# Brummi/BehindTheScenes

Measured on AMD Instinct MI355X. Metric: rendered rays/sec (192x640x64 samples), higher is better.
Workload: dtype f32 (lin_in as 3-term f16 split products on the f16 MFMA, f32 accumulate; everything else f32); 1 GPU; KITTI eval_depth.yaml forward, bs=1/GPU, 192x640, 2 views x 122880 rays, 64 samples/ray, nv=1, learn_empty=True (the yaml's effective default), want_weights+alphas, renderer only (feature-map encoder stand-in); samples_per_ray=64, parallelism=frames x1

## Files before the change

behindthescenes_amd/csrc/bts_common.h:

```cpp
#pragma once
#include <hip/hip_runtime.h>
#include <stdint.h>

#include "../../include/bts_render.h"

typedef float f32x16 __attribute__((ext_vector_type(16)));
typedef float f32x4 __attribute__((ext_vector_type(4)));
typedef float f32x2 __attribute__((ext_vector_type(2)));

#define BTS_EPS 1e-3f

namespace bts {

constexpr int kFwdWaves = 2;

constexpr int kNumFreqs = 6;
constexpr int kPeDim = 3 + 6 * kNumFreqs;

__device__ __forceinline__ void swap32(float& a, float& b) {
  auto r = __builtin_amdgcn_permlane32_swap(__float_as_uint(a), __float_as_uint(b), false, false);
  a = __uint_as_float(r[0]);
  b = __uint_as_float(r[1]);
}

// ... 157 lines not shown
  Taps t;
  t.w00 = (ex - ix) * (ey - iy);
  t.w01 = (ix - fx) * (ey - iy);
  t.w10 = (ex - ix) * (iy - fy);
  t.w11 = (ix - fx) * (iy - fy);
  x0 = (int)fx, y0 = (int)fy;
  x1 = min(x0 + 1, W - 1), y1 = min(y0 + 1, H - 1);
  x0 = max(0, min(x0, W - 1));
  y0 = max(0, min(y0, H - 1));
  x0 >>= fs, x1 >>= fs, y0 >>= fs, y1 >>= fs, W >>= fs;
  t.o00 = y0 * W + x0;
  t.o01 = y0 * W + x1;
  t.o10 = y1 * W + x0;
  t.o11 = y1 * W + x1;
  return t;
}

__device__ __forceinline__ Taps make_taps(float x, float y, int H, int W, int fs = 0) {
  int x0, y0, x1, y1;
  return make_taps_xy(x, y, H, W, x0, y0, x1, y1, fs);
}

__host__ __device__ inline int tile_cols(int Hm, int Wm, int blocks) { return (blocks && (Hm & 3) == 0 && (Wm & 15) == 0) ? (Wm >> 4) : 0; }
__device__ __forceinline__ unsigned tile_of(int y, int x, int Wm, int tw) {
  return tw ? (unsigned)((y >> 2) * tw + (x >> 4)) : (unsigned)(y * Wm + x) >> 6;
}
__device__ __forceinline__ int tile_base(int t, int Wm, int tw) {
  if (!tw) return t * 64;
  const int ty = t / tw;
  return ty * 4 * Wm + (t - ty * tw) * 16;
}
__device__ __forceinline__ int tile_rs(int Wm, int tw) { return tw ? Wm - 16 : 0; }
__device__ __forceinline__ int tile_px(int p0, int i, int rs) { return p0 + i + (i >> 4) * rs; }
__device__ __forceinline__ int tile_px_c(int p0, int cslot, int lslot, int rs) { return p0 + cslot + (cslot >> 4) * rs + lslot; }

__device__ __forceinline__ float depth_code(const Proj& pe, bool by_distance, bool inv_z, float inv_dmax, float inv_range, float d_min, float range) {
  const float v = by_distance ? pe.dist : pe.z;
  float r;
  if (inv_z) {
    const float vc = fmaxf(v, BTS_EPS);
    const float rv = div_by(1.0f, vc, by_distance ? __builtin_amdgcn_rcpf(vc) : pe.rz);
    r = div_by(rv - inv_dmax, inv_range, rcp_nr(inv_range));
  } else {
    r = div_by(v - d_min, range, rcp_nr(range));
  }
  return __builtin_fmaf(2.0f, r, -1.0f);
}

__device__ __forceinline__ float linspace_at(float start, float end, int steps, int i) {
  const float step = (end - start) / (float)(steps - 1);
  return i < steps / 2 ? start + step * (float)i : end - step * (float)(steps - i - 1);
}
__device__ __forceinline__ float coarse_base(int K, int k) { return K > 1 ? linspace_at(0.0f, 1.0f - 1.0f / (float)K, K, k) : 0.0f; }
__device__ __forceinline__ float coarse_depth(float u, float base, float step, float near, float far, bool lindisp) {
  const float sv = base + u * step;
  if (!lindisp) return near * (1.0f - sv) + far * sv;
  const float inv_near = div_by(1.0f, near, __builtin_amdgcn_rcpf(near)), inv_far = div_by(1.0f, far, __builtin_amdgcn_rcpf(far));
  const float den = inv_near * (1.0f - sv) + inv_far * sv;
  return div_by(1.0f, den, __builtin_amdgcn_rcpf(den));
}

template <int I>
__device__ __forceinline__ float pe_entry(const float (&v)[3], float freq_factor) {
  if constexpr (I < 3) {
    return v[I];
  } else if constexpr (I < kPeDim) {
    constexpr int j = I - 3;
    constexpr int oct = j / 6;
    constexpr int within = j % 6;
    constexpr int comp = within % 3;
    constexpr bool is_cos = within >= 3;
    const float f = freq_factor * (float)(1 << oct);
    float arg = v[comp] * f;
    if constexpr (is_cos) arg = arg + 1.57079637050628662109375f;
    return sinf(arg);
  } else if constexpr (I == kPeDim) {
    return 1.0f;
  } else {
    return 0.0f;
  }
}

__device__ __forceinline__ float relu1(float x) { return __builtin_amdgcn_fmed3f(x, 0.0f, 3.4028234663852886e38f); }

__device__ __forceinline__ int xcd_remap(int b, int nwg) {
  const int q = nwg >> 3, r = nwg & 7;
  const int xcd = b & 7, idx = b >> 3;
  return (xcd < r ? xcd * (q + 1) : r * (q + 1) + (xcd - r) * q) + idx;
}

__host__ __device__ constexpr int proj_storage_index(int hid) {
  const int ht = hid >> 5, r = hid & 31;
  const int q = r >> 3, h = (r >> 2) & 1, e = r & 3;
  return ht * 32 + h * 16 + q * 4 + e;
}
__host__ __device__ constexpr int proj_hidden_of_storage(int s) {
  const int ht = s >> 5, r = s & 31;
  const int h = r >> 4, q = (r >> 2) & 3, e = r & 3;
  return ht * 32 + 8 * q + 4 * h + e;
}

struct MlpLayout {
  int d_in, hd, nb;
  __host__ __device__ int w_in() const { return 0; }
  __host__ __device__ int b_in() const { return hd * d_in; }
  __host__ __device__ int blk(int i) const { return hd * d_in + hd + i * (2 * hd * hd + 2 * hd); }
  __host__ __device__ int blk_w0(int i) const { return blk(i); }
  __host__ __device__ int blk_b0(int i) const { return blk(i) + hd * hd; }
  __host__ __device__ int blk_w1(int i) const { return blk(i) + hd * hd + hd; }
  __host__ __device__ int blk_b1(int i) const { return blk(i) + 2 * hd * hd + hd; }
  __host__ __device__ int w_out() const { return blk(nb); }
  __host__ __device__ int b_out() const { return blk(nb) + hd; }
  __host__ __device__ int total() const { return blk(nb) + hd + 1; }
};

}
```

behindthescenes_amd/csrc/bts_field_kernel.h:

```cpp
#pragma once
#include "bts_common.h"
#include "bts_host.h"

#include <cstdio>
#include <cstring>

namespace bts {

struct FwdParams {
  const float* feat;
  const float* proj;
  const float* K_enc;
  const float* w2c_enc;
  const float* imgs;
  const float* K_r;
  const float* w2c_r;
  const float* empty_feature;
  const float* mlp;
  int n, H, W, nv;
  int fs;
  int enc_view;
  int code_mode, inv_z, learn_empty, empty_empty;
  float freq_factor, d_min, d_max;
  float inv_dmax, inv_range, range;
  const float* rays;
  const float* z_samp;
  const float* jitter;
  float* z_out;
  int lindisp;
  int Bp, K, hard_cap, white_bkgd;
  float* rgb;
  float* depth;
  float* weights;
  float* alphas;
  float* invalid;
  float* rgb_samps;
  float* sigma_raw;
  float* trans;
  float* invalid_wsum;
  float* invalid_any;
  const float* sigma_noise;
  union {
    const float* xyz;
    unsigned* sched;
  };
  union {
    float* q_sigma;
    const float* mlp_image;
  };
  int only_density;
  int tiles_per_sample;
  unsigned long long* dbg;
  int ablate;
  int lpr;
  int chunk_log2;
  int dyn_first;
  long groups;
};

struct PinnedSet {
  static constexpr int K = 64, nv = 1, fs = 0, enc_view = 0, lindisp = 1, empty_empty = 0, white_bkgd = 0;
  static constexpr int code_mode = 0, inv_z = 1, learn_empty = 1, hard_cap = 1;
  static bool matches(const FwdParams& p) {
    return p.lpr == 64 && p.K == K && p.nv == nv && p.fs == fs && p.enc_view == enc_view && !p.z_samp && p.jitter && !p.z_out && p.lindisp != 0 &&
           !p.sigma_noise && p.empty_empty == 0 && p.white_bkgd == 0 && p.code_mode == code_mode && p.inv_z != 0 && p.learn_empty != 0 &&
           p.hard_cap != 0 && p.rgb && p.depth && p.weights && p.alphas && p.invalid && !p.rgb_samps && !p.sigma_raw && !p.trans &&
           !p.invalid_wsum && !p.invalid_any;
  }
};

#ifdef BTS_PROBE
#define BTS_ABL(bit) ((p.ablate & (bit)) != 0)
#else
#define BTS_ABL(bit) false
#endif

template <int C, int HD, int NB, bool PROJ>
struct Lds {
  static constexpr int CF = PROJ ? 0 : C;
  static constexpr int KIN = CF + kPeDim + 1;
  static constexpr int W_IN = 0;
  static constexpr int BLK = W_IN + KIN * HD;
  static constexpr int BLK_STRIDE = 2 * HD * HD + 2 * HD;
  static constexpr int W_OUT = BLK + NB * BLK_STRIDE;
  static constexpr int EMPTY = W_OUT + HD;
  static constexpr int TOTAL = EMPTY + (PROJ ? HD : C);
};

template <int C>
__host__ __device__ constexpr int kernel_to_ref_input(int k) {
  if (k < C + 2) return k;
  if (k == C + 2) return C + 2;
  if (k == C + 3) return -1;
  return k - 1;
}

template <int C, int HD, int NB, bool PROJ>
__device__ __forceinline__ void stage_weights(float* lds, const float* __restrict__ mlp, const float* __restrict__ empty) {
  using L = Lds<C, HD, NB, PROJ>;
  constexpr int D_IN = C + kPeDim;
  const MlpLayout ml{D_IN, HD, NB};
  for (int i = threadIdx.x; i < L::KIN * HD; i += blockDim.x) {
    const int k = i / HD, hid = i % HD;
    const int src = kernel_to_ref_input<C>(k + (PROJ ? C : 0));
    lds[L::W_IN + i] = src >= 0 ? mlp[ml.w_in() + hid * D_IN + src] : mlp[ml.b_in() + hid];
  }
#pragma unroll
  for (int b = 0; b < NB; ++b) {
    float* base = lds + L::BLK + b * L::BLK_STRIDE;
    for (int i = threadIdx.x; i < HD * HD; i += blockDim.x) {
      const int k = i / HD, out = i % HD;
      base[i] = mlp[ml.blk_w0(b) + out * HD + k];
      base[HD * HD + HD + i] = mlp[ml.blk_w1(b) + out * HD + k];
    }
    for (int i = threadIdx.x; i < HD; i += blockDim.x) {
      base[HD * HD + i] = mlp[ml.blk_b0(b) + i];
      base[2 * HD * HD + HD + i] = mlp[ml.blk_b1(b) + i];
    }
  }
  for (int i = threadIdx.x; i < HD; i += blockDim.x) lds[L::W_OUT + i] = mlp[ml.w_out() + i];
  if constexpr (PROJ) {
    for (int hid = threadIdx.x; hid < HD; hid += blockDim.x) {
      float a = 0.0f;
      if (empty)
        for (int c = 0; c < C; ++c) a = __builtin_fmaf(mlp[ml.w_in() + hid * D_IN + c], empty[c], a);
      lds[L::EMPTY + hid] = a;
    }
  } else {
    for (int i = threadIdx.x; i < C; i += blockDim.x) lds[L::EMPTY + i] = empty ? empty[i] : 0.0f;
  }
}

struct GBuf {
  float4 v[2][4];
};

template <int HD>
__device__ __forceinline__ void gload(GBuf& b, const float4* __restrict__ G, const int (&o)[4], int tp2, int idx4) {
#pragma unroll
  for (int t = 0; t < 2; ++t) {
    const float4* row = G + (long)o[2 * tp2 + t] * (HD / 4) + idx4;
#pragma unroll
    for (int q = 0; q < 4; ++q) b.v[t][q] = row[q];
  }
}


template <bool FIRST>
__device__ __forceinline__ void gblend(f32x16& acc, const GBuf& b, float w0, float w1) {
  const f32x2 w0v = {w0, w0}, w1v = {w1, w1};
// ... 620 lines not shown
```

behindthescenes_amd/csrc/bts_render_iter.h:

```cpp
{
    constexpr bool SHARED = kTwoLoops && (BTS_ITER_SHARED);
    bool other_loop = false;
    const float nrec_in = nrec, z_pre_in = z_pre, zn_pre_in = zn_pre;
    auto q = kernarg_view<FwdParams>();
    asm volatile("" : "+s"(q));
    IterHead ih(q);
    const int K = BTS_PIN(PinnedSet::K, ih.K), H = ih.H, W = ih.W, nv = BTS_PIN(PinnedSet::nv, ih.nv), fs = BTS_PIN(PinnedSet::fs, ih.fs);
    long ray = lane_ray(g, 0);
    while (g >= sample_end) ++sample, sample_end += groups_per_sample;
    const Cam enc = load_cam(ih.w2c_enc + sample * 16, ih.K_enc + sample * 9);
    const float4* __restrict__ G = reinterpret_cast<const float4*>(ih.proj) + (long)sample * (H >> fs) * (W >> fs) * (HD / 4);
    float ox, oy, oz, dx, dy, dz, near = 0.0f, far = 0.0f;
    const bool from_jitter = BTS_PIN(true, ih.z_samp == nullptr);
    if constexpr (ONE_RAY) {
      ox = lane_value(nrec, 0), oy = lane_value(nrec, 1), oz = lane_value(nrec, 2), dx = lane_value(nrec, 3), dy = lane_value(nrec, 4);
      dz = lane_value(nrec, 5), near = lane_value(nrec, 6), far = lane_value(nrec, 7);
    } else {
      const float4 r0 = reinterpret_cast<const float4*>(ih.rays)[ray * 2];
      const float4 r1 = reinterpret_cast<const float4*>(ih.rays)[ray * 2 + 1];
      ox = r0.x, oy = r0.y, oz = r0.z, dx = r0.w, dy = r1.x, dz = r1.y, near = r1.z, far = r1.w;
    }
    const float* zsrc = from_jitter ? ih.jitter : ih.z_samp;
    const float* zrow = zsrc + ray * K;
    float z_cur = z_pre, zn_cur = zn_pre;
// ... 115 lines not shown
      } else {
        __builtin_amdgcn_fence(__ATOMIC_RELEASE, "wavefront");
        __builtin_amdgcn_wave_barrier();
        gl.tab[lane * 3 + 0] = (unsigned)tp.o00 * (HD * 4u), gl.tab[lane * 3 + 1] = (unsigned)tp.o01 * (HD * 4u), gl.tab[lane * 3 + 2] = (unsigned)tp.o10 * (HD * 4u);
        __builtin_amdgcn_fence(__ATOMIC_RELEASE, "wavefront");
        __builtin_amdgcn_wave_barrier();
        __builtin_amdgcn_fence(__ATOMIC_ACQUIRE, "wavefront");
        gl_prologue<HD, PINNED>(gl, rows, G, off_next, &taps);
      }
      {
        f32x16 bias[HT];
        {
          const float* bl = lh + LH::W_RAW + 3 * HD + 4 * h;
#pragma unroll
          for (int ht = 0; ht < HT; ++ht)
#pragma unroll
            for (int j = 0; j < 4; ++j) {
              const float4 v = *reinterpret_cast<const float4*>(bl + ht * 32 + 8 * j);
              bias[ht][4 * j + 0] = v.x, bias[ht][4 * j + 1] = v.y, bias[ht][4 * j + 2] = v.z, bias[ht][4 * j + 3] = v.w;
            }
        }
        SinCos3 raw;
        pe_direct(raw, v3, ih.freq_factor);
        __builtin_amdgcn_sched_barrier(0);
        int lane4 = lane * 4;
        asm volatile("" : "+v"(lane4));
        region_seq_l<HD, 0, SHARED, PINNED>(acc, gl, rows, G, wq, off_next, lh + LH::W_F16 + lane4, LH::TERM_STRIDE, raw, v3, ih.freq_factor, bias, h, &taps);
        if constexpr (NS > kNumFreqs) {
          g_step<HD, 12, SHARED, PINNED>(acc, gl, rows, G, wq, off_next, h, &taps), g_step<HD, 13, SHARED, PINNED>(acc, gl, rows, G, wq, off_next, h, &taps);
          g_step<HD, 14, SHARED, PINNED>(acc, gl, rows, G, wq, off_next, h, &taps), g_step<HD, 15, SHARED, PINNED>(acc, gl, rows, G, wq, off_next, h, &taps);
        }
      }
      if (BTS_PIN(PinnedSet::learn_empty, q->learn_empty) && __any(use_empty)) {
#pragma unroll
        for (int ht = 0; ht < HT; ++ht)
#pragma unroll
          for (int q = 0; q < 16; ++q) {
            const float ev = lh[LH::EMPTY + ht * 32 + mfma_row(q, 0) + 4 * h];
#pragma unroll
            for (int pt = 0; pt < 2; ++pt) acc[ht][pt][q] += emp[pt] ? ev : 0.0f;
          }
      }

      int lane4b = lane * 4;
      asm volatile("" : "+v"(lane4b));
#pragma unroll
      for (int b = 0; b < NB; ++b) {
        const float* base = lds + L::BLK + b * L::BLK_STRIDE;
        f32x16 net[HT][2];
#pragma unroll
        for (int ot = 0; ot < HT; ++ot)
#pragma unroll
          for (int q = 0; q < 16; ++q) {
            const int row = ot * 32 + mfma_row(q, 0) + 4 * h;
            const float bias = lh[LH::BIAS + b * 2 * HD + row];
            net[ot][0][q] = bias, net[ot][1][q] = bias;
          }
        if constexpr (HD == 32) hidden_layer_h(net, acc, lh + LH::W_BLK + (2 * b) * LH::BLK_LAYER_STRIDE + lane4b, LH::BLK_TERM_STRIDE, inv_scale);
        else hidden_layer<HD>(net, acc, base, lane);
#pragma unroll
        for (int ot = 0; ot < HT; ++ot)
#pragma unroll
          for (int q = 0; q < 16; ++q) {
            const int row = ot * 32 + mfma_row(q, 0) + 4 * h;
            const float bias = lh[LH::BIAS + b * 2 * HD + HD + row];
            acc[ot][0][q] += bias, acc[ot][1][q] += bias;
          }
        if constexpr (HD == 32) hidden_layer_h(acc, net, lh + LH::W_BLK + (2 * b + 1) * LH::BLK_LAYER_STRIDE + lane4b, LH::BLK_TERM_STRIDE, inv_scale);
        else hidden_layer<HD>(acc, net, base + HD * HD + HD, lane);
      }

      BTS_TICK(1)
      float p0 = 0.0f, p1 = 0.0f;
      if (BTS_ABL(32)) {
#pragma unroll
        for (int ht = 0; ht < HT; ++ht) p0 += acc[ht][0][0] + acc[ht][0][5] + acc[ht][0][15], p1 += acc[ht][1][0] + acc[ht][1][5] + acc[ht][1][15];
      } else {
        f32x2 pp = {0.0f, 0.0f};
#pragma unroll
        for (int ht = 0; ht < HT; ++ht)
#pragma unroll
          for (int q = 0; q < 16; ++q) {
            const float w2 = lds[L::W_OUT + ht * 32 + mfma_row(q, 0) + 4 * h];
            pp = __builtin_elementwise_fma((f32x2){w2, w2}, (f32x2){relu1(acc[ht][0][q]), relu1(acc[ht][1][q])}, pp);
          }
        p0 = pp[0], p1 = pp[1];
      }
      swap32(p0, p1);
      s_raw = __builtin_fmaf(p0 + p1, inv_scale, b_out);
      }
      float sigma = softplus(s_raw);
      if (BTS_PIN(PinnedSet::empty_empty, q->empty_empty)) sigma = pe.invalid ? 0.0f : sigma;
      if (BTS_PIN(false, q->sigma_noise != nullptr)) sigma += q->sigma_noise[ray * K + min(k, K - 1)];
      BTS_TICK(2)

      o_rgb = (OutP)q->rgb, o_depth = (OutP)q->depth, white_bkgd = BTS_PIN(PinnedSet::white_bkgd, q->white_bkgd);
      OutP o_weights = (OutP)q->weights, o_alphas = (OutP)q->alphas, o_invalid = (OutP)q->invalid;
      float *o_rgb_samps = BTS_PIN((float*)nullptr, q->rgb_samps), *o_sigma_raw = BTS_PIN((float*)nullptr, q->sigma_raw);
      float *o_trans = BTS_PIN((float*)nullptr, q->trans), *o_iw = BTS_PIN((float*)nullptr, q->invalid_wsum), *o_ia = BTS_PIN((float*)nullptr, q->invalid_any);
      if constexpr (PINNED) asm volatile("" : "+s"(o_rgb), "+s"(o_depth), "+s"(o_weights), "+s"(o_alphas), "+s"(o_invalid));
      else
      asm volatile("" : "+s"(o_rgb), "+s"(o_depth), "+s"(o_weights), "+s"(o_alphas), "+s"(o_invalid), "+s"(o_rgb_samps), "+s"(o_sigma_raw), "+s"(o_trans),
                   "+s"(o_iw), "+s"(o_ia));

#pragma unroll
      for (int j = 0; j < NVMAX; ++j) col[3 * j] = col[3 * j + 1] = col[3 * j + 2] = 0.0f, inv[j] = pe.invalid;
      if (nv > 0 && !BTS_ABL(8)) {
#pragma unroll
        for (int j0 = 0; j0 < NVMAX; j0 += 4) {
          constexpr int NB4 = NVMAX < 4 ? NVMAX : 4;
          Taps tcs[NB4];
          bool invs[NB4];
#pragma unroll
          for (int b = 0; b < NB4; ++b) {
            const int jj = min(j0 + b, nv - 1);
            tcs[b] = tp_enc, invs[b] = pe.invalid;
            if (jj != BTS_PIN(PinnedSet::enc_view, q->enc_view)) {
              const Cam cj = load_cam(q->w2c_r + ((long)sample * nv + jj) * 16, q->K_r + ((long)sample * nv + jj) * 9);
              const Proj pc = project<false>(cj, px, py, pz);
              tcs[b] = make_taps(pc.x, pc.y, H, W);
              invs[b] = pc.invalid | pe.invalid;
            }
          }
          float4 tex[NB4][4];
#pragma unroll
          for (int b = 0; b < NB4; ++b) {
            const float4* img = reinterpret_cast<const float4*>(q->imgs) + ((long)sample * nv + min(j0 + b, nv - 1)) * H * W;
            tex[b][0] = img[tcs[b].o00], tex[b][1] = img[tcs[b].o01], tex[b][2] = img[tcs[b].o10], tex[b][3] = img[tcs[b].o11];
          }
          if constexpr (NB4 > 1) __builtin_amdgcn_sched_barrier(0);
#pragma unroll
          for (int b = 0; b < NB4; ++b) {
            const int j = j0 + b;
            const Taps& tc = tcs[b];
            const float4 a = tex[b][0], bb = tex[b][1], cc = tex[b][2], d = tex[b][3];
            const float c0 = ((a.x * tc.w00 + bb.x * tc.w01) + cc.x * tc.w10) + d.x * tc.w11;
            const float c1 = ((a.y * tc.w00 + bb.y * tc.w01) + cc.y * tc.w10) + d.y * tc.w11;
            const float c2 = ((a.z * tc.w00 + bb.z * tc.w01) + cc.z * tc.w10) + d.z * tc.w11;
            if (j < nv) col[3 * j + 0] = c0, col[3 * j + 1] = c1, col[3 * j + 2] = c2, inv[j] = invs[b];
          }
        }
      }

      const float delta = (k + 1 < K) ? (z_nx - z) : 1e10f;
      float alpha = 1.0f - transmittance(delta, sigma);
      if (BTS_PIN(PinnedSet::hard_cap, q->hard_cap) && k == K - 1) alpha = 1.0f;
      const float t = valid ? (1.0f - alpha) + 1e-10f : 1.0f;
      const float incl = seg_scan_mul(t, lpr, kl);
      float excl = dpp_f<kDppWaveShr1>(1.0f, incl);
      if (kl == 0) excl = 1.0f;
      const float T = (pk48 ? (mainl ? 1.0f : Tc_D) : T_carry) * excl;
      if (pk48) Tc_D = Tc_D * __builtin_bit_cast(float, __builtin_amdgcn_readlane(__builtin_bit_cast(int, incl), 63));
      if (ONE_RAY && K > 64) T_carry = T_carry * __builtin_bit_cast(float, __builtin_amdgcn_readlane(__builtin_bit_cast(int, incl), 63));
      const float wgt = valid ? alpha * T : 0.0f;
      BTS_TICK(3)
      if constexpr (EPI) {
        float ws[NVMAX], any[NVMAX];
        const unsigned long long seg = pk48 ? (mainl ? 0x0000FFFFFFFFFFFFull : 0xFFFF000000000000ull)
                                            : (lpr == 64 ? ~0ull : (((1ull << lpr) - 1ull) << ((lane | (lpr - 1)) - (lpr - 1))));
#pragma unroll
        for (int j = 0; j < NVMAX; ++j) {
          ws[j] = seg_scan_add((valid && inv[j]) ? wgt : 0.0f, lpr, kl);
          const unsigned long long hit = __ballot(valid && inv[j]);
          any[j] = (hit & seg) ? 1.0f : 0.0f;
        }
        if (pk48 ? (lane == 47 || lane == 63) : kl == lpr - 1) {
          const bool more = pk48 ? (!mainl && it > 0) : kc > 0;
          const long idx = ray * nv;
          if (nv == NVMAX && NVMAX % 4 == 0 && !more) {
#pragma unroll
            for (int j4 = 0; j4 < NVMAX / 4; ++j4) {
              if (o_iw) reinterpret_cast<float4*>(o_iw + idx)[j4] = make_float4(ws[4 * j4], ws[4 * j4 + 1], ws[4 * j4 + 2], ws[4 * j4 + 3]);
              if (o_ia) reinterpret_cast<float4*>(o_ia + idx)[j4] = make_float4(any[4 * j4], any[4 * j4 + 1], any[4 * j4 + 2], any[4 * j4 + 3]);
            }
          } else {
#pragma unroll
            for (int j = 0; j < NVMAX; ++j)
              if (j < nv) {
                if (o_iw) o_iw[idx + j] = (more ? o_iw[idx + j] : 0.0f) + ws[j];
                if (o_ia) o_ia[idx + j] = more ? fmaxf(o_ia[idx + j], any[j]) : any[j];
              }
          }
        }
      }
      depth_part = depth_part + wgt * z;
      w_part = w_part + wgt;
#pragma unroll
      for (int i = 0; i < NVMAX * 3; ++i) rgb_part[i] = rgb_part[i] + wgt * col[i];
      if (valid && !BTS_ABL(16)) {
        const long pk = ray * K + k;
        if constexpr (PINNED) {
          __builtin_nontemporal_store(wgt, &(o_weights + ray * K)[(unsigned)k]), __builtin_nontemporal_store(alpha, &(o_alphas + ray * K)[(unsigned)k]);
          __builtin_nontemporal_store(inv[0] ? 1.0f : 0.0f, &(o_invalid + ray * K)[(unsigned)k]);
        }
        if (BTS_PIN(false, o_weights != nullptr)) o_weights[pk] = wgt;
        if (BTS_PIN(false, o_alphas != nullptr)) o_alphas[pk] = alpha;
        if (o_sigma_raw) o_sigma_raw[pk] = s_raw;
        if (o_trans) o_trans[pk] = T;
        if (BTS_PIN(false, o_invalid != nullptr)) {
#pragma unroll
          for (int j = 0; j < NVMAX; ++j)
            if (j < nv) o_invalid[pk * nv + j] = inv[j] ? 1.0f : 0.0f;
        }
        if (o_rgb_samps) {
          float* dst = o_rgb_samps + pk * (nv * 3);
          if (nv == NVMAX && (NVMAX * 3) % 4 == 0) {
#pragma unroll
            for (int i = 0; i < NVMAX * 3 / 4; ++i)
              reinterpret_cast<float4*>(dst)[i] = make_float4(col[4 * i], col[4 * i + 1], col[4 * i + 2], col[4 * i + 3]);
          } else if (nv == NVMAX && (NVMAX * 3) % 2 == 0) {
#pragma unroll
            for (int i = 0; i < NVMAX * 3 / 2; ++i) reinterpret_cast<float2*>(dst)[i] = make_float2(col[2 * i], col[2 * i + 1]);
          } else {
#pragma unroll
            for (int i = 0; i < NVMAX * 3; ++i)
              if (i < nv * 3) dst[i] = col[i];
          }
        }
      }
      if (pk48) {
        const float dsum = seg_scan_add(depth_part, 48, kl), wsum = seg_scan_add(w_part, 48, kl);
        float csum[NVMAX * 3];
#pragma unroll
        for (int i = 0; i < NVMAX * 3; ++i) csum[i] = i < nv * 3 ? seg_scan_add(rgb_part[i], 48, kl) : 0.0f;
        if (lane == 47 || (lane == 63 && it == 2)) {
          o_depth[ray] = dsum;
#pragma unroll
          for (int i = 0; i < NVMAX * 3; ++i)
            if (i < nv * 3) o_rgb[ray * nv * 3 + i] = white_bkgd ? (csum[i] + 1.0f) - wsum : csum[i];
        }
      }
// ... 31 lines not shown
```

behindthescenes_amd/csrc/bts_render_kernel.h:

```cpp
#pragma once
#include "bts_field_kernel.h"

namespace bts {

#ifdef BTS_PROBE
#define BTS_TICK(i)                                                  \
  if (p.ablate & 128) {                                              \
    const unsigned long long t_now = __builtin_readcyclecounter();   \
    t_acc[i] += t_now - t_last;                                      \
    t_last = t_now;                                                  \
  }
#else
#define BTS_TICK(i)
#endif

template <int CTRL, int ROW_MASK = 0xF>
__device__ __forceinline__ float dpp_f(float old, float src) {
  return __builtin_bit_cast(float, __builtin_amdgcn_update_dpp(__builtin_bit_cast(int, old), __builtin_bit_cast(int, src), CTRL,
                                                               ROW_MASK, 0xF, false));
}
constexpr int kDppRowShr = 0x110;
constexpr int kDppWaveShr1 = 0x138;
constexpr int kDppWaveShl1 = 0x130;
constexpr int kDppBcast15 = 0x142;
constexpr int kDppBcast31 = 0x143;

__device__ __forceinline__ float seg_scan_mul(float x, int lpr, int kl) {
  float y;
  if (lpr == 48) {
    x *= dpp_f<kDppRowShr + 1>(1.0f, x);
    x *= dpp_f<kDppRowShr + 2>(1.0f, x);
    x *= dpp_f<kDppRowShr + 4>(1.0f, x);
    x *= dpp_f<kDppRowShr + 8>(1.0f, x);
    x *= dpp_f<kDppBcast15, 0x2>(1.0f, x);
    x *= dpp_f<kDppBcast31, 0x4>(1.0f, x);
    return x;
  }
  if (lpr >= 16) {
    x *= dpp_f<kDppRowShr + 1>(1.0f, x);
    x *= dpp_f<kDppRowShr + 2>(1.0f, x);
    x *= dpp_f<kDppRowShr + 4>(1.0f, x);
    x *= dpp_f<kDppRowShr + 8>(1.0f, x);
  } else {
    y = dpp_f<kDppRowShr + 1>(1.0f, x), x *= (kl >= 1) ? y : 1.0f;
    y = dpp_f<kDppRowShr + 2>(1.0f, x), x *= (kl >= 2) ? y : 1.0f;
    y = dpp_f<kDppRowShr + 4>(1.0f, x), x *= (kl >= 4) ? y : 1.0f;
  }
  if (lpr >= 32) x *= dpp_f<kDppBcast15, 0xA>(1.0f, x);
  if (lpr >= 64) x *= dpp_f<kDppBcast31, 0xC>(1.0f, x);
  return x;
}
__device__ __forceinline__ float seg_scan_add(float x, int lpr, int kl) {
  float y;
  if (lpr == 48) {
    x += dpp_f<kDppRowShr + 1>(0.0f, x);
    x += dpp_f<kDppRowShr + 2>(0.0f, x);
    x += dpp_f<kDppRowShr + 4>(0.0f, x);
    x += dpp_f<kDppRowShr + 8>(0.0f, x);
    x += dpp_f<kDppBcast15, 0x2>(0.0f, x);
    x += dpp_f<kDppBcast31, 0x4>(0.0f, x);
    return x;
  }
  if (lpr >= 16) {
    x += dpp_f<kDppRowShr + 1>(0.0f, x);
    x += dpp_f<kDppRowShr + 2>(0.0f, x);
    x += dpp_f<kDppRowShr + 4>(0.0f, x);
    x += dpp_f<kDppRowShr + 8>(0.0f, x);
  } else {
    y = dpp_f<kDppRowShr + 1>(0.0f, x), x += (kl >= 1) ? y : 0.0f;
    y = dpp_f<kDppRowShr + 2>(0.0f, x), x += (kl >= 2) ? y : 0.0f;
    y = dpp_f<kDppRowShr + 4>(0.0f, x), x += (kl >= 4) ? y : 0.0f;
  }
  if (lpr >= 32) x += dpp_f<kDppBcast15, 0xA>(0.0f, x);
  if (lpr >= 64) x += dpp_f<kDppBcast31, 0xC>(0.0f, x);
  return x;
}

typedef _Float16 h8 __attribute__((ext_vector_type(8)));
typedef unsigned u32x4 __attribute__((ext_vector_type(4)));

template <int C, int HD, int NB>
struct LdsH {
  static constexpr int HT = HD / 32;
  static constexpr int W_RAW = 0;
  static constexpr int W_F16 = W_RAW + 4 * HD;
  static constexpr int TERM_STRIDE = 3 * HT * 64 * 4;
  static constexpr int BIAS = W_F16 + 2 * TERM_STRIDE;
  static constexpr int EMPTY = BIAS + NB * 2 * HD;
  static constexpr int SCALE = EMPTY + HD;
  static constexpr int W_BLK = SCALE + 4;
  static constexpr int BLK_TERM_STRIDE = 2 * 64 * 4;
  static constexpr int BLK_LAYER_STRIDE = 2 * BLK_TERM_STRIDE;
  static constexpr int TOTAL = W_BLK + NB * 2 * BLK_LAYER_STRIDE;
};

template <int C, int HD, int NB>
__device__ __forceinline__ void stage_weights_h(float* lh, const float* empty_proj, const float* __restrict__ mlp) {
  using LH = LdsH<C, HD, NB>;
  constexpr int HT = HD / 32;
  constexpr int D_IN = C + kPeDim;
  const MlpLayout ml{D_IN, HD, NB};
  int* mx = reinterpret_cast<int*>(lh + LH::SCALE + 2);
  if (threadIdx.x == 0) *mx = 0;
  __syncthreads();
  float m = 0.0f;
  for (int i = threadIdx.x; i < 39 * HD; i += blockDim.x) m = fmaxf(m, fabsf(mlp[ml.w_in() + (i % HD) * D_IN + C + i / HD]));
  for (int i = threadIdx.x; i < NB * 2 * HD * HD; i += blockDim.x) {
    const int b = i / (2 * HD * HD), j = i % (2 * HD * HD);
    m = fmaxf(m, fabsf(mlp[(j < HD * HD ? ml.blk_w0(b) : ml.blk_w1(b)) + j % (HD * HD)]));
  }
  atomicMax(mx, __float_as_int(m));
  __syncthreads();
  const float wmax = __int_as_float(*mx);
  int ex = 0;
  if (wmax > 0.0f && wmax < 3.0e38f) frexpf(wmax, &ex);
  const int S = max(-40, min(40, 14 - ex));
  const float scale = ldexpf(1.0f, S);
  if (threadIdx.x == 0) lh[LH::SCALE] = scale, lh[LH::SCALE + 1] = ldexpf(1.0f, -S);
  for (int i = threadIdx.x; i < 4 * HD; i += blockDim.x) {
    const int k = i / HD, hid = i % HD;
    lh[LH::W_RAW + i] = (k < 3 ? mlp[ml.w_in() + hid * D_IN + C + k] : mlp[ml.b_in() + hid]) * scale;
  }
  _Float16* wf = reinterpret_cast<_Float16*>(lh + LH::W_F16);
  for (int i = threadIdx.x; i < 3 * HT * 64 * 8; i += blockDim.x) {
    const int e = i & 7, lane = (i >> 3) & 63, ht = (i >> 9) % HT, r = i / (HT * 512);
    const int slot = 8 * (lane >> 5) + e, hid = ht * 32 + (lane & 31);
    float w = 0.0f;
    if (slot < 12) w = mlp[ml.w_in() + hid * D_IN + C + 3 + 6 * (2 * r + slot / 6) + slot % 6] * scale;
    else if (r == 0 && slot < 14) w = mlp[ml.w_in() + hid * D_IN + C + (slot - 12)] * scale;
    else if (r == 1 && slot == 12) w = mlp[ml.w_in() + hid * D_IN + C + 2] * scale;
    asm("" : "+v"(w));
    const _Float16 hi = (_Float16)w;
// ... 362 lines not shown
template <int HD, int R, bool SH = false, bool PIN = false>
__device__ __forceinline__ void region_seq_l(f32x16 (&acc)[HD / 32][2], const GatherLds& gl, GRows& rows, const float4* __restrict__ G,
                                             const float (&wq)[2][4], unsigned (&off_next)[4], const float* wf, int term_stride, SinCos3& raw,
                                             const float (&v3)[3], float ff, const f32x16* bias, int h = 0, GTapRegs* taps = nullptr) {
  static_assert(R == 0, "entered at region 0");
  SinCos3 pre;
  region_seq_li<HD, 0, SH, PIN>(acc, gl, rows, G, wq, off_next, wf, term_stride, raw, pre, v3, ff, bias, h, taps);
}

template <int C, int HD, int NB>
__device__ __attribute__((noinline)) float eval_point_exact(const float* lds, const float4* G, const float* w2c, const float* Kc, int H, int W,
                                                            int fs, int code_mode, int inv_z, float inv_dmax, float inv_range, float d_min, float range,
                                                            float freq_factor, int learn_empty, float b_out, float px, float py, float pz) {
  FwdParams q;
  q.H = H, q.W = W, q.fs = fs, q.code_mode = code_mode, q.inv_z = inv_z, q.inv_dmax = inv_dmax, q.inv_range = inv_range, q.d_min = d_min;
  q.range = range, q.freq_factor = freq_factor, q.learn_empty = learn_empty, q.ablate = 0;
  const Cam enc = load_cam(w2c, Kc);
  Proj pe;
  return eval_point<C, HD, NB, true>(q, lds, enc, G, (int)(threadIdx.x & 63), b_out, px, py, pz, pe);
}

template <bool PIN>
struct IterHeadT {
  const float* w2c_enc;
  const float* K_enc;
  const float* proj;
  const float* rays;
  const float* z_samp;
  const float* jitter;
  int K, H, W, nv, fs, code_mode, inv_z, learn_empty;
  float inv_dmax, inv_range, d_min, range, freq_factor;
  template <typename Q>
  __device__ __forceinline__ explicit IterHeadT(Q q) {
    const FwdParams __attribute__((address_space(4)))* f = head_of(q);
    w2c_enc = f->w2c_enc, K_enc = f->K_enc, proj = f->proj, rays = f->rays, z_samp = f->z_samp, jitter = f->jitter;
    K = f->K, H = f->H, W = f->W, nv = f->nv, fs = f->fs, code_mode = f->code_mode, inv_z = f->inv_z, learn_empty = f->learn_empty;
    inv_dmax = f->inv_dmax, inv_range = f->inv_range, d_min = f->d_min, range = f->range, freq_factor = f->freq_factor;
    if constexpr (PIN)
    asm volatile("" : "+s"(w2c_enc), "+s"(K_enc), "+s"(proj), "+s"(rays), "+s"(z_samp), "+s"(K), "+s"(H), "+s"(W), "+s"(nv), "+s"(fs),
                 "+s"(code_mode), "+s"(inv_z), "+s"(learn_empty), "+s"(inv_dmax), "+s"(inv_range), "+s"(d_min), "+s"(range), "+s"(freq_factor));
  }
  static __device__ __forceinline__ const FwdParams __attribute__((address_space(4)))* head_of(const FwdParams __attribute__((address_space(4)))* q) { return q; }
  template <typename B>
  static __device__ __forceinline__ const FwdParams __attribute__((address_space(4)))* head_of(const B __attribute__((address_space(4)))* q) { return &q->f; }
};
using IterHead = IterHeadT<false>;

__device__ __forceinline__ void store4(float* p, const float4& v) { *reinterpret_cast<float4*>(p) = v; }
__device__ __forceinline__ void store4(float __attribute__((address_space(1)))* p, const float4& v) {
  *(f32x4 __attribute__((address_space(1)))*)p = (f32x4){v.x, v.y, v.z, v.w};
}

#define BTS_PIN(constant, field) (PINNED ? (constant) : (field))
template <int C, int HD, int NB, int NVMAX, bool ONE_RAY, bool F16, bool EPI = false, bool DYN = false, bool IMG = false, bool PINNED = false>
__global__ __launch_bounds__(256, kFwdWaves) void render_kernel_p(const FwdParams p) {
  static_assert(F16, "lin_in runs on the f16 matrix pipe in split precision: the fp32-input-MFMA form of rounds 1 - 2 is gone (git history)");
  static_assert(!PINNED || (ONE_RAY && !EPI && DYN && IMG && NB == 0 && NVMAX == PinnedSet::nv), "the pinned set is the evaluation frame's");
  using OutP = std::conditional_t<PINNED, float __attribute__((address_space(1)))*, float*>;
  using L = Lds<C, HD, NB, true>;
  using LH = LdsH<C, HD, NB>;
  constexpr int HT = HD / 32;
  constexpr int NS = 4 * HT;
  __shared__ __attribute__((aligned(16))) float lds[L::TOTAL + LH::TOTAL + 4];
  float* const lh = lds + ((L::TOTAL + 3) & ~3);
#ifdef BTS_PROBE
  const unsigned long long t_entry = __builtin_readcyclecounter();
#endif
  if constexpr (IMG) {
    const float4* src = reinterpret_cast<const float4*>(p.mlp_image);
    float4* dst = reinterpret_cast<float4*>(lds);
    for (int i = threadIdx.x; i < MlpImage<C, HD, NB>::FLOATS / 4; i += 256) dst[i] = src[i];
    __syncthreads();
  } else {
    stage_weights<C, HD, NB, true>(lds, p.mlp, p.empty_feature);
    __syncthreads();
    stage_weights_h<C, HD, NB>(lh, lds + L::EMPTY, p.mlp);
    __syncthreads();
  }
#ifdef BTS_PROBE
  const unsigned long long t_stage = __builtin_readcyclecounter() - t_entry;
#endif
  const float scale = __builtin_bit_cast(float, __builtin_amdgcn_readfirstlane(__builtin_bit_cast(int, lh[LH::SCALE])));
  const float inv_scale = __builtin_bit_cast(float, __builtin_amdgcn_readfirstlane(__builtin_bit_cast(int, lh[LH::SCALE + 1])));

  const int lane = threadIdx.x & 63;
  const int h0 = lane >> 5;
  const int wave = __builtin_amdgcn_readfirstlane(threadIdx.x >> 6);
  extern __shared__ __attribute__((aligned(128))) char gather_lds[];
  GatherLds gl;
  {
    char* base = gather_lds + wave * kGatherLdsPerWave;
    gl.ring = base;
    gl.ring_m0 = (unsigned)(unsigned long)base;
    gl.tab = reinterpret_cast<unsigned*>(base + 3 * 4096);
    gl.m = lane >> 3;
    gl.piece16 = 16u * (unsigned)(((lane & 7) + (lane >> 4)) & 7);
    gl.piece16x = gl.piece16 ^ 64u;
    const int col = lane & 31;
#pragma unroll
    for (int q = 0; q < 4; ++q) gl.rd[q] = (unsigned)(col * 128 + ((4 * h0 + q - (col >> 1)) & 7) * 16);
  }
  const int nwg = gridDim.x;
  const int wg = xcd_remap(blockIdx.x, nwg);
  const int wg_per_xcd = nwg >> 3;
  const int xcd = wg / wg_per_xcd;
  const int lw = (wg - xcd * wg_per_xcd) * 4 + wave;
  const int waves_per_xcd = wg_per_xcd * 4;
  const int lpr = ONE_RAY ? 64 : p.lpr;
  const bool pk48 = !ONE_RAY && lpr == 48;
  const bool mainl = lane < 48;
  const int R = pk48 ? 4 : 64 / lpr;
  const int kl = pk48 ? (mainl ? lane : lane - 48) : lane & (lpr - 1);
  auto lane_ray = [&](int gg, int it) -> long { return pk48 ? (long)gg * 4 + (mainl ? it : 3) : (long)gg * R + lane / lpr; };
  auto lane_k = [&](int it) -> int { return pk48 && !mainl ? 16 * it + kl : kl; };
  const int CHL = p.chunk_log2;
  const int n_groups = (int)p.groups;
  const int n_chunks = (n_groups + (1 << CHL) - 1) >> CHL;
  auto group_of = [&](int idx) -> int {
    const int c = ((idx >> CHL) << 3) + xcd;
    const int gg = (c << CHL) + (idx & ((1 << CHL) - 1));
    return (c < n_chunks && gg < n_groups) ? gg : -1;
  };
  const int Bp = p.Bp;
  const float b_out = as_const(p.mlp)[MlpLayout{C + kPeDim, HD, NB}.b_out()];
  const int lane_off0 = h0 * HD + (lane & 31);

#ifdef BTS_PROBE
  unsigned long long t_acc[8] = {0, 0, 0, 0, 0, 0, 0, 0};
  unsigned long long t_last = __builtin_readcyclecounter();
  const unsigned long long t_begin = t_last;
  unsigned hw_id = 0, xcc_id = 0;
  asm volatile("s_getreg_b32 %0, hwreg(HW_REG_HW_ID)" : "=s"(hw_id));
  asm volatile("s_getreg_b32 %0, hwreg(HW_REG_XCC_ID, 0, 4)" : "=s"(xcc_id));
#endif
  const int groups_per_sample = Bp / R;
  int sample_end = groups_per_sample;
  int sample = 0;
  int idx = lw;
  int g = group_of(idx);
  int g_nx = -1;
  unsigned pend = 0u;
  auto n_static = [&]() -> int { return kernarg_view<FwdParams>()->dyn_first >> 3; };
  auto claim = [&]() -> unsigned {
    unsigned t = 0u;
    if (lane == 0) t = atomicAdd(kernarg_view<FwdParams>()->sched + 32 * xcd, 1u);
    return t;
  };
  auto claimed_group = [&](unsigned ticket) -> int { return group_of(n_static() + (int)__builtin_amdgcn_readfirstlane(ticket)); };
  auto next_group = [&]() -> int {
    const int gn = g_nx;
    if (gn >= 0) {
      const int ns = n_static();
      g_nx = idx + waves_per_xcd < ns ? group_of(idx + waves_per_xcd) : claimed_group(pend);
      if (g_nx >= 0 && idx + 2 * waves_per_xcd >= ns) pend = claim();
    }
    return gn;
  };
  if constexpr (DYN) {
    const int ns = n_static();
    g = idx < ns ? group_of(idx) : claimed_group(claim());
    if (g >= 0) g_nx = idx + waves_per_xcd < ns ? group_of(idx + waves_per_xcd) : claimed_group(claim());
    if (g_nx >= 0 && idx + 2 * waves_per_xcd >= ns) pend = claim();
  }
  float z_pre = 0.0f, zn_pre = 0.0f;
  if (g >= 0) {
    const int K = BTS_PIN(PinnedSet::K, p.K);
// ... 83 lines not shown
```

Before: 353.6 million rays/s.

## Trim pinned-path ALU: cheaper ReLU, 12-byte texel loads, inline-asm DPP scan

On the pinned fast path the output layer's ReLU becomes x+|x|, with the doubling folded into the output scale by subtracting one from the exponent of inv_scale. Image texel fetches switch to 3-float loads through 32-bit unsigned offsets, and a guard on H*W keeps those offsets from overflowing. The transmittance product scan becomes a hand-written inline-asm DPP sequence with s_nop padding. The aim is fewer VALU instructions and less load traffic. Risks are the exponent trick misbehaving for denormal or zero scales and the inline asm hiding instructions from the compiler's scheduler.

```diff
diff --git a/behindthescenes_amd/csrc/bts_common.h b/behindthescenes_amd/csrc/bts_common.h
--- a/behindthescenes_amd/csrc/bts_common.h
+++ b/behindthescenes_amd/csrc/bts_common.h
@@ -263,6 +263,7 @@
 }
 
 __device__ __forceinline__ float relu1(float x) { return __builtin_amdgcn_fmed3f(x, 0.0f, 3.4028234663852886e38f); }
+__device__ __forceinline__ float relu2(float x) { return x + __builtin_fabsf(x); }
 
 __device__ __forceinline__ int xcd_remap(int b, int nwg) {
   const int q = nwg >> 3, r = nwg & 7;
diff --git a/behindthescenes_amd/csrc/bts_field_kernel.h b/behindthescenes_amd/csrc/bts_field_kernel.h
--- a/behindthescenes_amd/csrc/bts_field_kernel.h
+++ b/behindthescenes_amd/csrc/bts_field_kernel.h
@@ -65,7 +65,8 @@
     return p.lpr == 64 && p.K == K && p.nv == nv && p.fs == fs && p.enc_view == enc_view && !p.z_samp && p.jitter && !p.z_out && p.lindisp != 0 &&
            !p.sigma_noise && p.empty_empty == 0 && p.white_bkgd == 0 && p.code_mode == code_mode && p.inv_z != 0 && p.learn_empty != 0 &&
            p.hard_cap != 0 && p.rgb && p.depth && p.weights && p.alphas && p.invalid && !p.rgb_samps && !p.sigma_raw && !p.trans &&
-           !p.invalid_wsum && !p.invalid_any;
+           !p.invalid_wsum && !p.invalid_any &&
+           (long)p.H * p.W * 16 < (1L << 32);
   }
 };
 
diff --git a/behindthescenes_amd/csrc/bts_render_iter.h b/behindthescenes_amd/csrc/bts_render_iter.h
--- a/behindthescenes_amd/csrc/bts_render_iter.h
+++ b/behindthescenes_amd/csrc/bts_render_iter.h
@@ -221,12 +221,14 @@
 #pragma unroll
           for (int q = 0; q < 16; ++q) {
             const float w2 = lds[L::W_OUT + ht * 32 + mfma_row(q, 0) + 4 * h];
+            if constexpr (PINNED) pp = __builtin_elementwise_fma((f32x2){w2, w2}, (f32x2){relu2(acc[ht][0][q]), relu2(acc[ht][1][q])}, pp);
+            else
             pp = __builtin_elementwise_fma((f32x2){w2, w2}, (f32x2){relu1(acc[ht][0][q]), relu1(acc[ht][1][q])}, pp);
           }
         p0 = pp[0], p1 = pp[1];
       }
       swap32(p0, p1);
-      s_raw = __builtin_fmaf(p0 + p1, inv_scale, b_out);
+      s_raw = __builtin_fmaf(p0 + p1, inv_scale_out, b_out);
       }
       float sigma = softplus(s_raw);
       if (BTS_PIN(PinnedSet::empty_empty, q->empty_empty)) sigma = pe.invalid ? 0.0f : sigma;
@@ -265,6 +267,15 @@
 #pragma unroll
           for (int b = 0; b < NB4; ++b) {
             const float4* img = reinterpret_cast<const float4*>(q->imgs) + ((long)sample * nv + min(j0 + b, nv - 1)) * H * W;
+            if constexpr (PINNED) {
+              const auto* base = (const char __attribute__((address_space(1)))*)img;
+              auto texel = [&](int o) {
+                typedef float f32x3 __attribute__((ext_vector_type(3)));
+                const f32x3 v = *(const f32x3 __attribute__((address_space(1)))*)(base + (unsigned)o * 16u);
+                return make_float4(v[0], v[1], v[2], 0.0f);
+              };
+              tex[b][0] = texel(tcs[b].o00), tex[b][1] = texel(tcs[b].o01), tex[b][2] = texel(tcs[b].o10), tex[b][3] = texel(tcs[b].o11);
+            } else
             tex[b][0] = img[tcs[b].o00], tex[b][1] = img[tcs[b].o01], tex[b][2] = img[tcs[b].o10], tex[b][3] = img[tcs[b].o11];
           }
           if constexpr (NB4 > 1) __builtin_amdgcn_sched_barrier(0);
@@ -285,7 +296,9 @@
       float alpha = 1.0f - transmittance(delta, sigma);
       if (BTS_PIN(PinnedSet::hard_cap, q->hard_cap) && k == K - 1) alpha = 1.0f;
       const float t = valid ? (1.0f - alpha) + 1e-10f : 1.0f;
-      const float incl = seg_scan_mul(t, lpr, kl);
+      float incl;
+      if constexpr (PINNED) incl = scan_mul_wave(t);
+      else incl = seg_scan_mul(t, lpr, kl);
       float excl = dpp_f<kDppWaveShr1>(1.0f, incl);
       if (kl == 0) excl = 1.0f;
       const float T = (pk48 ? (mainl ? 1.0f : Tc_D) : T_carry) * excl;
diff --git a/behindthescenes_amd/csrc/bts_render_kernel.h b/behindthescenes_amd/csrc/bts_render_kernel.h
--- a/behindthescenes_amd/csrc/bts_render_kernel.h
+++ b/behindthescenes_amd/csrc/bts_render_kernel.h
@@ -48,6 +48,17 @@
   }
   if (lpr >= 32) x *= dpp_f<kDppBcast15, 0xA>(1.0f, x);
   if (lpr >= 64) x *= dpp_f<kDppBcast31, 0xC>(1.0f, x);
+  return x;
+}
+__device__ __forceinline__ float scan_mul_wave(float x) {
+  asm("s_nop 1\n\tv_mul_f32_dpp %0, %0, %0 row_shr:1 row_mask:0xf bank_mask:0xf\n\t"
+      "s_nop 1\n\tv_mul_f32_dpp %0, %0, %0 row_shr:2 row_mask:0xf bank_mask:0xf\n\t"
+      "s_nop 1\n\tv_mul_f32_dpp %0, %0, %0 row_shr:4 row_mask:0xf bank_mask:0xf\n\t"
+      "s_nop 1\n\tv_mul_f32_dpp %0, %0, %0 row_shr:8 row_mask:0xf bank_mask:0xf\n\t"
+      "s_nop 1\n\tv_mul_f32_dpp %0, %0, %0 row_bcast:15 row_mask:0xa bank_mask:0xf\n\t"
+      "s_nop 1\n\tv_mul_f32_dpp %0, %0, %0 row_bcast:31 row_mask:0xc bank_mask:0xf\n\t"
+      "s_nop 1"
+      : "+v"(x));
   return x;
 }
 __device__ __forceinline__ float seg_scan_add(float x, int lpr, int kl) {
@@ -576,6 +587,7 @@
 #endif
   const float scale = __builtin_bit_cast(float, __builtin_amdgcn_readfirstlane(__builtin_bit_cast(int, lh[LH::SCALE])));
   const float inv_scale = __builtin_bit_cast(float, __builtin_amdgcn_readfirstlane(__builtin_bit_cast(int, lh[LH::SCALE + 1])));
+  const float inv_scale_out = PINNED ?__builtin_bit_cast(float, __builtin_bit_cast(int, inv_scale) - (1 << 23)) : inv_scale;
 
   const int lane = threadIdx.x & 63;
   const int h0 = lane >> 5;
```

Result: no change. 356.7 million rays/s (median of 6 runs) (+0.9%).
